# Stanford-ILIAD/Diverse-Conventions

Hardware: NVIDIA B200
Metric: agent-steps/sec (env+obs) (higher is better)
Workload: dtype u8

## Files before the change

diverse_conventions_b200/csrc/policy_kernels.cu:

```cuda
#include <cuda_bf16.h>
#include <cuda_runtime.h>
#include <stdint.h>
#include <stdlib.h>
#include <string.h>

#include <new>
#include <vector>

#include "api_common.h"
#include "oc_core.cuh"
#include "oc_device.cuh"
#include "mixed_schedule.h"
#include "ocb.h"
#include "policy_internal.h"

using namespace ocb;

namespace {

constexpr int kRows = 128;
constexpr int kHid = 64;
constexpr int kCo = 32;
constexpr int kSlots = 16;
constexpr int kK1 = 9 * kSlots;
// ... 480 lines not shown
                if (round > 0) mbar_wait_p<kProf>(bars + 8 * (PB_W_EMPTY + slot), (round - 1) & 1, pw[PW_W_EMPTY]);
                if (load) {
                    if (elect_one()) {
                        mbar_arrive_expect_tx(bars + 8 * (PB_W_FULL + slot), kChunk);
                        bulk_g2s(s_wring + slot * kChunk, (g ? blob_c : blob_a) + L.head_bytes + (size_t)j * kChunk, kChunk,
                                 bars + 8 * (PB_W_FULL + slot));
                    }
                    __syncwarp();
                }
                if (++slot == Reff) slot = 0, ++round;
            }
        }
    }
}

template <bool kProf, int kNet>
__device__ __forceinline__ void pair_conv_role(long long* pw, const PolicyParams& prm, int t0, int t1, const BlobLayout L, uint32_t tmem,
                                               uint32_t a_head, uint32_t bars, const int cp0 = 0, const int cpstep = 1,
                                               const uint32_t ring = kColRing, const int col_full = PB_COL_FULL,
                                               const int col_empty = PB_COL_EMPTY) {
    const int W = prm.W, H = prm.H, PH = H - 2, npos = prm.npos;
    constexpr int kN = kNet < 0 ? kHid : kCo;
    const uint32_t idesc = make_idesc(kRows, kN);
    const uint32_t a_wchi = a_head + (kNet == 1 ? kPConvBytes : 0), a_wclo = a_wchi + 2 * kPConvBytes;
    const int b_full = kNet < 0 ? PB_D1_FULL : PBS_D1_FULL + 2 * kNet, b_empty = kNet < 0 ? PB_D1_EMPTY : PBS_D1_EMPTY + 2 * kNet;
    uint32_t head_gen = 0, u = 0;
    uint32_t uses[2] = {0, 0};
    const bool tracer = kNet <= 0;
    uint32_t t_slot = 0, t_round = 0;
    auto advance = [&](uint32_t& slot, uint32_t& round, int n) {
        for (int i = 0; i < n; ++i)
            if (++slot == ring) slot = 0, ++round;
    };

    for (int t = t0; t < t1; ++t, ++u) {
        if (blob_changed(prm, t, t0)) {
            mbar_wait_p<kProf>(bars + 8 * PB_HEAD_FULL, head_gen & 1, pw[PW_HEAD_FULL]);
            ++head_gen;
        }
        if (kNet == 1) {
            const int s_last = (npos - 1) & 1;
            const uint32_t cum = (u + 1) * (uint32_t)((npos + 1 - s_last) / 2);
            mbar_wait_p<kProf>(bars + 8 * (PBS_D1_FULL + s_last), (cum - 1) & 1, pw[PW_D3_FULL]);
        }
        uint32_t w_slot = t_slot, w_round = t_round;
        uint32_t r_slot = t_slot;
        uint32_t c_slot = t_slot;
        int cols_seen = 0, released = 0, ox = 0, oy = cp0;
        while (oy >= PH) oy -= PH, ++ox, c_slot = (c_slot + 1 == ring) ? 0 : c_slot + 1;
        for (int cp = cp0; cp < npos; cp += cpstep) {
            const int st = cp & 1;
            for (; cols_seen < ox + 3; ++cols_seen) {
                mbar_wait_p<kProf>(bars + 8 * (col_full + w_slot), w_round & 1, pw[PW_COL_FULL]);
                if (++w_slot == ring) w_slot = 0, ++w_round;
// ... 7 lines not shown
            uint32_t n_slot = c_slot;
            while (noy >= PH) noy -= PH, ++nox, n_slot = (n_slot + 1 == ring) ? 0 : n_slot + 1;
            const int keep = cp + cpstep < npos ? nox : W;
            const uint32_t s1 = (c_slot + 1 >= ring) ? c_slot + 1 - ring : c_slot + 1;
            const uint32_t s2 = (c_slot + 2 >= ring) ? c_slot + 2 - ring : c_slot + 2;
            const uint32_t cellb = tmem + kColCells + (uint32_t)oy * kCellCols, colw = (uint32_t)H * kCellCols;
            const uint32_t cb0 = cellb + c_slot * colw, cb1 = cellb + s1 * colw, cb2 = cellb + s2 * colw;
            const long long ti0 = kProf ? clock64() : 0;
            if (cp == 3 && tracer) trace_ev<kProf>(prm, t - t0, 54);
            if (cp < 2 && tracer) trace_ev<kProf>(prm, t - t0, 11 + cp);
            if (elect_one()) {
#pragma unroll
                for (int j = 0; j < 9; ++j) {
                    const int dx = j / 3, dy = j - dx * 3;
                    const uint32_t ta = (dx == 0 ? cb0 : dx == 1 ? cb1 : cb2) + dy * kCellCols;
                    umma_bf16_ts(d1, ta, make_desc(a_wchi + j * 256, 128, 2304), idesc, j > 0);
                    umma_bf16_ts(d1, ta, make_desc(a_wclo + j * 256, 128, 2304), idesc, 1);
                }
                umma_commit(bars + 8 * (b_full + st));
                uint32_t rs = r_slot;
                for (int c = released; c < keep; ++c) {
                    umma_commit(bars + 8 * (col_empty + rs));
                    rs = (rs + 1 == ring) ? 0 : rs + 1;
                }
                if (cp + cpstep >= npos) umma_commit(bars + 8 * (PB_HEAD_EMPTY + (u & 1)));
            }
            __syncwarp();
            for (; released < keep; ++released) r_slot = (r_slot + 1 == ring) ? 0 : r_slot + 1;
            if (kProf) pw[PW_ISSUE_CONV] += clock64() - ti0;
            if (cp < 8 && tracer) trace_ev<kProf>(prm, t - t0, 16 + cp);
            ++uses[st];
            ox = nox, oy = noy, c_slot = n_slot;
// ... 142 lines not shown
            if (half == 1) {
                tc_fence_before();
                mbar_arrive(bars + 8 * (PB_D3_EMPTY + g));
            }
            head_accumulate(net, v, s_b2 + half * 32, s_wh, half * 32, head);
        }
        mbar_arrive(bars + 8 * (PB_HEAD_EMPTY + (u & 1)));
        if (kProf && (warp & 3) == 0) trace_ev<kProf>(prm, trace_vt, g == 0 ? 50 : 53);
        out(t, trow_id, net, head, drawn);
        if (kProf && warp == 0) trace_ev<kProf>(prm, trace_vt, 51);
    }
}
constexpr int kSColD3 = kPColD2 + kHid;
constexpr int kSHeadGroup = 1;

template <bool kProf>
__device__ __forceinline__ void single_fc_role(long long* pw, const PolicyParams& prm, int t0, int t1, const BlobLayout L, uint32_t tmem,
                                               uint32_t a_wring, uint32_t bars) {
    const int npos = prm.npos;
    const int R = prm.pair_ring, nch = L.chunks;
    const bool resident = R >= nch;
    const bool static_w = resident && prm.tile_policy == nullptr;
    const int Reff = resident ? nch : R;
    const uint32_t idesc = make_idesc(kRows, kHid);
    uint32_t u = 0, w_gen = 0, wround = 0;
    uint32_t cnt0 = 0, cnt1 = 0;
    int slot = 0;
    for (int t = t0; t < t1; ++t, ++u) {
        const bool chg = blob_changed(prm, t, t0);
        const bool w_loaded = !resident || chg;
        if (resident && w_loaded) ++w_gen;
        for (int j = 0; j < npos + 2; ++j) {
            const int sg = j < npos ? (j & 1) : (j - npos);
            const uint32_t k = sg ? cnt1 : cnt0;
            mbar_wait_p<kProf>(bars + 8 * (PB_A2_FULL + sg), k & 1, pw[PW_A2_FULL]);
            if (sg) ++cnt1; else ++cnt0;
            if (j == npos && u > 0) mbar_wait_p<kProf>(bars + 8 * PB_D3_EMPTY, (u - 1) & 1, pw[PW_D3_FULL]);
            if (w_loaded) mbar_wait_p<kProf>(bars + 8 * (PB_W_FULL + slot), resident ? ((w_gen - 1) & 1) : (wround & 1), pw[PW_W_FULL]);
            tc_fence_after();
            const uint32_t dst = tmem + (j < npos ? kPColD2 : kSColD3);
            const bool first = (j == 0 || j == npos);
            const uint32_t a_hi = tmem + kPColA2 + sg * kA2Cols, a_lo = a_hi + 16;
            const uint32_t b_hi = a_wring + slot * kChunk, b_lo = b_hi + 4096;
            const long long tf0 = kProf ? clock64() : 0;
            if (elect_one()) {
#pragma unroll
// ... 3 lines not shown
                    umma_bf16_ts(dst, a_hi + ks * 8, blo, idesc, 1);
                    umma_bf16_ts(dst, a_lo + ks * 8, bhi, idesc, 1);
                }
                umma_commit(bars + 8 * (PB_A2_EMPTY + sg));
                if (!static_w) umma_commit(bars + 8 * (PB_W_EMPTY + slot));
                if (j == npos - 1) umma_commit(bars + 8 * PB_D2_FULL);
                if (j == npos + 1) umma_commit(bars + 8 * PB_D3_FULL);
            }
            __syncwarp();
            if (kProf) pw[PW_ISSUE_FC] += clock64() - tf0;
            if (++slot >= Reff) slot = 0, ++wround;
        }
    }
}

template <bool kProf, class Out>
__device__ __forceinline__ void single_epilogue_role(long long* pw, const PolicyParams& prm, int t0, int t1, const BlobLayout L,
                                                     uint32_t tmem, const uint8_t* s_head, uint32_t bars, Out&& out) {
    const int warp = threadIdx.x >> 5, g = warp >> 2, trow_id = (warp & 3) * 32 + (threadIdx.x & 31);
    const int npos = prm.npos;
    const int net = prm.single == 2 ? 1 : 0;
    const uint32_t trow = tmem + ((uint32_t)((warp & 3) * 32) << 16);
    const uint8_t* rest = s_head + kPRestOff - L.bias1;
    const float* s_bias1 = reinterpret_cast<const float*>(rest + L.bias1);
    const float* s_b1 = reinterpret_cast<const float*>(rest + L.b1);
    const float* s_b2 = reinterpret_cast<const float*>(rest + L.b2);
    const float* s_wh = reinterpret_cast<const float*>(rest + L.wh);
    const float* s_bh = reinterpret_cast<const float*>(rest + L.bh);
    uint32_t u = 0, head_gen = 0, pubs = 0, d1_uses = 0;
    auto publish = [&](float (&v)[32], const float* bias) {
        const uint32_t a2 = trow + kPColA2 + g * kA2Cols;
        const float4* b4 = reinterpret_cast<const float4*>(bias);
        uint32_t hi[16], lo[16];
#pragma unroll
        for (int q = 0; q < 8; ++q) {
            const float4 b = b4[q];
            split2(fmaxf(v[4 * q] + b.x, 0.0f), fmaxf(v[4 * q + 1] + b.y, 0.0f), hi[2 * q], lo[2 * q]);
            split2(fmaxf(v[4 * q + 2] + b.z, 0.0f), fmaxf(v[4 * q + 3] + b.w, 0.0f), hi[2 * q + 1], lo[2 * q + 1]);
        }
        if (pubs >= 1) {
            mbar_wait_p<kProf>(bars + 8 * (PB_A2_EMPTY + g), (pubs - 1) & 1, pw[PW_A2_EMPTY]);
            tc_fence_after();
        }
        tmem_st16(a2, hi);
        tmem_st16(a2 + 16, lo);
        tmem_st_wait();
        tc_fence_before();
        mbar_arrive(bars + 8 * (PB_A2_FULL + g));
        ++pubs;
    };
    for (int t = t0; t < t1; ++t, ++u) {
        if (blob_changed(prm, t, t0)) {
            mbar_wait_p<kProf>(bars + 8 * PB_HEAD_FULL, head_gen & 1, pw[PW_HEAD_FULL]);
            ++head_gen;
        }
        for (int j = g; j < npos; j += 2, ++d1_uses) {
            mbar_wait_p<kProf>(bars + 8 * (PBS_D1_FULL + g), d1_uses & 1, pw[PW_D1_FULL]);
            tc_fence_after();
            float v[32];
            tmem_ld32(trow + kPColD1 + g * kCo, v);
            tc_fence_before();
            mbar_arrive(bars + 8 * (PBS_D1_EMPTY + g));
            publish(v, s_bias1 + j * kCo);
        }
        mbar_wait_p<kProf>(bars + 8 * PB_D2_FULL, u & 1, pw[PW_D2_FULL]);
        tc_fence_after();
        {
            float v[32];
            tmem_ld32(trow + kPColD2 + g * 32, v);
// ... 271 lines not shown
    }
    const int smem_max = kSmemBudget + 128;
    if (err == cudaSuccess) err = cudaFuncSetAttribute(policy_pair_kernel<false>, cudaFuncAttributeMaxDynamicSharedMemorySize, smem_max);
    if (err == cudaSuccess) err = cudaFuncSetAttribute(policy_pair_kernel<true>, cudaFuncAttributeMaxDynamicSharedMemorySize, smem_max);
    if (err == cudaSuccess) err = cudaFuncSetAttribute(rollout_fused_kernel<false, false, 1>, cudaFuncAttributeMaxDynamicSharedMemorySize, smem_max);
    if (err == cudaSuccess) err = cudaFuncSetAttribute(rollout_fused_kernel<true, false, 1>, cudaFuncAttributeMaxDynamicSharedMemorySize, smem_max);
    if (err == cudaSuccess) err = cudaFuncSetAttribute(rollout_fused_kernel<false, true, 1>, cudaFuncAttributeMaxDynamicSharedMemorySize, smem_max);
    if (err == cudaSuccess) err = cudaFuncSetAttribute(rollout_fused_kernel<true, true, 1>, cudaFuncAttributeMaxDynamicSharedMemorySize, smem_max);
    if (err == cudaSuccess) err = cudaFuncSetAttribute(rollout_fused_kernel<false, false, 2>, cudaFuncAttributeMaxDynamicSharedMemorySize, smem_max);
    if (err == cudaSuccess) err = cudaFuncSetAttribute(rollout_fused_kernel<true, false, 2>, cudaFuncAttributeMaxDynamicSharedMemorySize, smem_max);
    if (err == cudaSuccess) err = cudaFuncSetAttribute(rollout_fused_kernel<false, false, 1, true>, cudaFuncAttributeMaxDynamicSharedMemorySize, smem_max);
    if (err == cudaSuccess) err = cudaFuncSetAttribute(rollout_fused_kernel<false, true, 1, true>, cudaFuncAttributeMaxDynamicSharedMemorySize, smem_max);
    if (err == cudaSuccess) err = cudaFuncSetAttribute(rollout_fused_kernel<false, false, 2, true>, cudaFuncAttributeMaxDynamicSharedMemorySize, smem_max);
    if (err == cudaSuccess) err = cudaFuncSetAttribute(rollout_fused_kernel<false, false, 1, false, true>, cudaFuncAttributeMaxDynamicSharedMemorySize, smem_max);
    if (err == cudaSuccess) err = cudaFuncSetAttribute(rollout_fused_kernel<false, false, 2, false, true>, cudaFuncAttributeMaxDynamicSharedMemorySize, smem_max);
    if (err == cudaSuccess) err = cudaFuncSetAttribute(conv512_kernel, cudaFuncAttributeMaxDynamicSharedMemorySize, smem_max);
    if (err == cudaSuccess) err = cudaFuncSetAttribute(gemm512_kernel<false, false>, cudaFuncAttributeMaxDynamicSharedMemorySize, smem_max);
    if (err == cudaSuccess) err = cudaFuncSetAttribute(gemm512_kernel<true, true>, cudaFuncAttributeMaxDynamicSharedMemorySize, smem_max);
    if (err != cudaSuccess) {
        cudaGetLastError();
        ocb_policy_destroy(p);
        return fail(OCB_ERR_CUDA, "ocb_policy_create: %s", cudaGetErrorString(err));
    }
    *out = p;
    return OCB_OK;
}

static int set_weights512(ocb_policy* p, int policy, int net, const float* conv_w, const float* conv_b, const float* fc1_w,
                          const float* fc1_b, const float* fc2_w, const float* fc2_b, const float* head_w, const float* head_b) {
    const Blob5& L = p->L5;
// ... 355 lines not shown
    if (tile_policy == nullptr && (policy_index < 0 || policy_index >= p->n_policies)) return fail(OCB_ERR_INVALID_ARG, "policy index out of range");
    if (mixed && (mix->partner_policy < 0 || mix->partner_policy >= p->n_policies))
        return fail(OCB_ERR_INVALID_ARG, "policy index out of range");
    if (env_w != p->W || env_h != p->H) return fail(OCB_ERR_INVALID_ARG, "env and policy were built for different layouts");
    if (T < 1) return fail(OCB_ERR_INVALID_ARG, "T must be >= 1");
    if (mixed && (mix->L < 2 || T != 2 * mix->L || envp.N % (mix->L - 1) != 0))
        return fail(OCB_ERR_INVALID_ARG, "mixed play runs T = 2 L steps over a multiple of L - 1 worlds");
    if (mixed && (obs_slab == nullptr || actions == nullptr)) return fail(OCB_ERR_INVALID_ARG, "obs_buf and actions are required");
    if (!cross && !mixed && (obs_slab == nullptr || actions == nullptr || values == nullptr))
        return fail(OCB_ERR_INVALID_ARG, "obs_slab, actions and values are required");
    if (cross && (envp.N % kRows) != 0)
        return fail(OCB_ERR_INVALID_ARG, "cross-play needs a multiple of %d worlds (one weight set per 128-row tile of a seat), got %d", kRows, envp.N);
    if (population && (envp.N % kRows) != 0)
        return fail(OCB_ERR_INVALID_ARG, "population self-play needs a multiple of %d worlds (one weight set per slice), got %d", kRows, envp.N);
    if (cross && values != nullptr) return fail(OCB_ERR_INVALID_ARG, "the cross-play rollout runs no critic: values must be NULL");
    const int wtiles = (envp.N + kFWorlds - 1) / kFWorlds;
    int slots = 1;
    {
        const int fixed2 = fused_smem_layout(p->npos, 0, p->S, p->SC, 2).total;
        const bool fits2 = fixed2 <= kSmemBudget && (kSmemBudget - fixed2) / kChunk >= 4;
        const char* e = getenv("OCB_FUSED_SLOTS");
        const bool want2 = e != nullptr ? (e[0] == '2') : (wtiles > p->sm_count);
        if (want2 && fits2) slots = 2;
    }
    const int fixed = fused_smem_layout(p->npos, 0, p->S, p->SC, slots).total;
    int ring = (kSmemBudget - fixed) / kChunk;
    if (ring > kPMaxRing) ring = kPMaxRing;
    if (ring > 2 * p->L.chunks) ring = 2 * p->L.chunks;
    if (fixed > kSmemBudget || ring < 4)
        return fail(OCB_ERR_UNSUPPORTED, "layout too large for the fused rollout kernel (%d x %d)", p->W, p->H);
    DeviceGuard guard(p->device);
    FusedParams fp;
    memset(&fp, 0, sizeof(fp));
    fp.pol.blobs = tile_policy != nullptr ? p->d_blobs : p->d_blobs + (size_t)policy_index * 2 * (size_t)p->L.total;
    fp.pol.blob_stride = (size_t)p->L.total;
    fp.pol.W = p->W, fp.pol.H = p->H, fp.pol.S = p->S, fp.pol.SC = p->SC, fp.pol.npos = p->npos;
    fp.pol.M = kRows, fp.pol.tiles = 1;
    fp.pol.deterministic = deterministic, fp.pol.seed = seed, fp.pol.offset = 0;
    fp.pol.rng_rows_per_seat = p->rng_rows_per_seat, fp.pol.rng_add0 = p->rng_add0, fp.pol.rng_add1 = p->rng_add1;
    fp.pol.d_offset = reinterpret_cast<const unsigned long long*>(d_offset);
    fp.pol.net_mask = 3, fp.pol.pair_ring = ring, fp.pol.stage_stride = p->stage_stride;
    fp.pol.tile_policy = tile_policy, fp.pol.f_vt_round = slots * (T + 1), fp.pol.f_slots = slots;
    fp.pol.f_seat1_tiles = population ? 0 : envp.N / kRows;
    fp.env = envp;
    fp.T = T, fp.wtiles = wtiles, fp.slots = slots, fp.cross = cross ? 1 : 0;
    fp.obs_slab = obs_slab, fp.actions = actions, fp.logp = logp, fp.values = values, fp.reward = reward, fp.done = done;
    if (mixed) {
        fp.mix_L = mix->L, fp.mix_seed = mix->mix_seed, fp.mix_partner_seed = mix->partner_seed;
        fp.mix_partner_blobs = p->d_blobs + (size_t)mix->partner_policy * 2 * (size_t)p->L.total;
    }
    const int groups = (wtiles + slots - 1) / slots;
    const int ctas = groups < p->sm_count ? groups : p->sm_count;
    const size_t smem = (size_t)fused_smem_layout(p->npos, ring, p->S, p->SC, slots).total;
    fp.pol.trace = d_trace, fp.pol.trace_u0 = trace_u0, fp.pol.trace_n = trace_n;
    {
        const char* e = getenv("OCB_FUSED_VEC_LOADER");
        fp.vec_loader = e != nullptr ? (e[0] != '0') : (p->SC % 16 == 0);
    }
    {
        const int cols = 192 / (kCellCols * p->H);
        const char* e = getenv("OCB_FUSED_SPLIT");
        const bool want = e != nullptr ? (e[0] != '0') : true;
        fp.col_ring = (want && slots == 1 && !cross && !mixed && cols >= p->W) ? (p->W < kFMaxColRing ? p->W : kFMaxColRing) : 0;
        if (fp.col_ring < p->W) fp.col_ring = 0;
    }
    const cudaStream_t st = (cudaStream_t)stream;
    if (mixed) {
        fp.col_ring = kColRing;
        if (slots == 2)
            rollout_fused_kernel<false, false, 2, false, true><<<ctas, kFThreads, smem, st>>>(fp);
        else
            rollout_fused_kernel<false, false, 1, false, true><<<ctas, kFThreads, smem, st>>>(fp);
    } else if (population) {
        if (fp.col_ring > 0) {
            rollout_fused_kernel<false, true, 1, true><<<ctas, kFThreads, smem, st>>>(fp);
        } else {
            fp.col_ring = kColRing;
            if (slots == 2)
                rollout_fused_kernel<false, false, 2, true><<<ctas, kFThreads, smem, st>>>(fp);
            else
                rollout_fused_kernel<false, false, 1, true><<<ctas, kFThreads, smem, st>>>(fp);
        }
    } else if (fp.col_ring > 0) {
        if (d_trace != nullptr)
            rollout_fused_kernel<true, true, 1><<<ctas, kFThreads, smem, st>>>(fp);
        else
            rollout_fused_kernel<false, true, 1><<<ctas, kFThreads, smem, st>>>(fp);
// ... 22 lines not shown
```

diverse_conventions_b200/csrc/rollout_fused.cuh:

```cuda
#pragma once

struct FusedParams {
    PolicyParams pol;
    RolloutParams env;
    int T;
    int wtiles;
    int8_t* obs_slab;
    int32_t* actions;
    float* logp;
    float* values;
    int32_t* reward;
    int32_t* done;
    int vec_loader;
    int col_ring;
    int slots;
    int cross;
    int mix_L;
    unsigned long long mix_seed, mix_partner_seed;
    const uint8_t* mix_partner_blobs;
};

constexpr int kFEnvWarps = 2;
constexpr int kFWarpConvC = kPWarpProd + 1;
constexpr int kFWarpEnv = kFWarpConvC + 1;
constexpr int kFThreads = 32 * (kFWarpEnv + kFEnvWarps);
constexpr int kFWorlds = 32 * kFEnvWarps;
constexpr int kFMaxColRing = 6;
enum : int {
    FB_OBS_FULL = PB_COUNT,
    FB_OBS_EMPTY = PB_COUNT + 2,
    FB_ACT_FULL = PB_COUNT + 4,
    FB_COL_FULL = PB_COUNT + 6,
    FB_COL_EMPTY = FB_COL_FULL + kFMaxColRing,
    FB_COUNT = FB_COL_EMPTY + kFMaxColRing
};
static_assert((int)FB_COUNT <= (int)PB_TMEM_SLOT, "barrier block overflow");

struct FusedSmemLayout {
    int head, wring, bars, act, tables, tmpl, envw;
    int view_stride, env_warp_bytes, slot_bytes, total;
};
__host__ __device__ inline FusedSmemLayout fused_smem_layout(int npos, int ring, int S, int SC, int slots) {
// ... 26 lines not shown
    __device__ __forceinline__ void next() {
        if (two && s == 0) {
            s = 1;
            return;
        }
        s = 0;
        if (++u > T) u = 0, kt0 += stride, two = slots == 2 && kt0 + 1 < wtiles;
    }
};
__host__ __device__ inline int fused_virtual_tiles(int wtiles, int slots, int grid, int cta, int T) {
    int n = 0;
    for (int kt0 = cta * slots; kt0 < wtiles; kt0 += grid * slots) n += ((slots == 2 && kt0 + 1 < wtiles) ? 2 : 1) * (T + 1);
    return n;
}

template <bool kProf, bool kSplit>
__device__ __forceinline__ void fused_loader_role(const FusedParams& fp, uint32_t nvt, uint32_t tmem, const uint8_t* s_env,
                                                  const FusedSmemLayout& sl, uint32_t bars) {
    const int lwarp = (threadIdx.x >> 5) - kEpiWarps, lg = lwarp >> 2, lw = lwarp & 3, lane = threadIdx.x & 31;
    const int W = fp.pol.W, H = fp.pol.H, seg = 5 * H;
    const uint32_t* myrow0 = reinterpret_cast<const uint32_t*>(s_env + (lw & 1) * sl.env_warp_bytes + (lw >> 1) * sl.view_stride +
                                                               lane * fp.pol.SC);
    const uint32_t* myrow = myrow0;
    const uint32_t tcells = tmem + ((uint32_t)(lw * 32) << 16) + kColCells;
    const uint32_t ncols = nvt * (uint32_t)W;
    uint32_t lt = 0;
    int lx = lg;
    bool fresh = true;
    FusedCursor cur(fp);
    uint32_t seen[2] = {0, 0};
    for (uint32_t gc = lg; gc < ncols; gc += 2) {
        if (fresh) {
            myrow = myrow0 + cur.s * (sl.slot_bytes >> 2);
            mbar_wait(bars + 8 * (FB_OBS_FULL + cur.s), (cur.s ? seen[1] : seen[0]) & 1);
            if (kProf && lwarp == 0) trace_ev<kProf>(fp.pol, (int)lt, 8);
        }
        const bool first_col = fresh;
        fresh = false;
        const uint32_t ring = kSplit ? (uint32_t)fp.col_ring : (uint32_t)kColRing;
        const int slot = gc % ring;
        if (gc >= ring) {
            mbar_wait(bars + 8 * ((kSplit ? FB_COL_EMPTY : PB_COL_EMPTY) + slot), ((gc / ring) - 1) & 1);
            tc_fence_after();
        }
        if (fp.vec_loader) {
            const uint32_t* colp = myrow + lx * seg;
            const int r = (int)((reinterpret_cast<uintptr_t>(colp) >> 2) & 3);
            const uint4* src4 = reinterpret_cast<const uint4*>(colp - r);
            constexpr int kMaxVec = (5 * kMaxH + 3 + 3) / 4;
// ... 33 lines not shown
                for (int q = 0; q < 5; ++q) w[q] = mine[y * 5 + q];
                const uint4 c0 = make_uint4(bytes_bf16x2(w[0], pair_sel(0, 1)), bytes_bf16x2(w[0], pair_sel(2, 3)),
                                            bytes_bf16x2(w[1], pair_sel(0, 1)), bytes_bf16x2(w[1], pair_sel(2, 3)));
                const uint4 c1 = make_uint4(bytes_bf16x2(w[2], pair_sel(0, 1)), bytes_bf16x2(w[4], pair_sel(0, 1)),
                                            bytes_bf16x2(w[4], pair_sel(2, 3)), bytes_bf16x2(w[3], pair_sel(3, 4)));
                tmem_st8(tcells + (slot * H + y) * kCellCols, c0, c1);
            }
        }
        tmem_st_wait();
        tc_fence_before();
        mbar_arrive(bars + 8 * ((kSplit ? FB_COL_FULL : PB_COL_FULL) + slot));
        if (kProf && lwarp == 0 && first_col) trace_ev<kProf>(fp.pol, (int)lt, 9);
        if (kProf && lw == 0 && lx >= 1 && lx <= 4) trace_ev<kProf>(fp.pol, (int)lt, 3 + lx);
        lx += 2;
        if (lx >= W) {
            mbar_arrive(bars + 8 * (FB_OBS_EMPTY + cur.s));
            if (kProf && lwarp == 0) trace_ev<kProf>(fp.pol, (int)lt, 10);
            if (cur.s) ++seen[1]; else ++seen[0];
            cur.next();
            lx -= W, ++lt, fresh = true;
        }
    }
}

__device__ __forceinline__ void bulk_wait_read_1() { asm volatile("cp.async.bulk.wait_group.read 1;" ::: "memory"); }

template <int P>
struct FusedSlot {
    World<P> w;
    int cur_return, ep_add;
    long long ret_add;
    int n, nbytes;
    int j;
    bool valid, tma_ok, tma_pending;
    int8_t* obs_ptr;
    int32_t *rew_ptr, *done_ptr;
    uint32_t vts, acts;
};

template <bool kProf, int kSlots, bool kMix = false>
__device__ __forceinline__ void fused_env_role(const FusedParams& fp, uint8_t* s_env, const FusedSmemLayout& sl, const Tables& tb,
                                               const uint8_t* tmpl, const uint8_t* s_act, uint32_t bars) {
    constexpr int P = 2;
    const int ew = (threadIdx.x >> 5) - kFWarpEnv, lane = threadIdx.x & 31;
    const Consts c = load_consts(tb);
    const int SC = tb.SC, N = fp.env.N, T = fp.T;
    const int view_stride = sl.view_stride;
    const size_t PN = (size_t)P * N, obs_view_stride = (size_t)N * SC, obs_step_stride = PN * SC;
    const bool store_obs = fp.obs_slab != nullptr;

    FusedSlot<P> sa, sb;
    StepPre2 pre;
    sa.vts = sa.acts = sb.vts = sb.acts = 0;
    sa.tma_pending = sb.tma_pending = false;

    auto planes_of = [&](int slot) { return s_env + slot * sl.slot_bytes + ew * sl.env_warp_bytes; };
    auto objs_of = [&](int slot) { return reinterpret_cast<uint16_t*>(planes_of(slot) + (size_t)P * view_stride) + lane; };

    auto begin_tile = [&](FusedSlot<P>& q, int slot, int kt) {
        const int n0 = kt * kFWorlds + ew * 32;
        q.n = n0 + lane;
        q.valid = q.n < N;
        const int nl = q.valid ? q.n : N - 1;
        q.nbytes = max(0, min(32, N - n0)) * SC;
        q.obs_ptr = store_obs ? fp.obs_slab + (size_t)n0 * SC : nullptr;
        q.tma_ok = store_obs && fp.env.use_tma && q.nbytes > 0 && ((q.nbytes & 15) == 0) &&
                   ((reinterpret_cast<uintptr_t>(q.obs_ptr) & 15u) == 0) && ((obs_view_stride & 15u) == 0);
        q.rew_ptr = fp.reward ? fp.reward + q.n : nullptr;
        q.done_ptr = fp.done ? fp.done + q.n : nullptr;
        if constexpr (kMix) {
            q.j = q.n % (fp.mix_L - 1);
            q.tma_ok = store_obs && fp.env.use_tma && (SC & 15) == 0 && (reinterpret_cast<uintptr_t>(fp.obs_slab) & 15u) == 0;
        }
        load_world<P, 1, 8>(tb, c, fp.env, nl, 0, objs_of(slot), q.w);
        q.cur_return = fp.env.cur_return[nl];
// ... 14 lines not shown
                bulk_wait_read_all();
            } else if (lane == 0) {
                if (other_pending)
                    bulk_wait_read_1();
                else
                    bulk_wait_read_all();
            }
            q.tma_pending = false;
        }
        if (u > 0) {
            __syncwarp();
#pragma unroll
            for (int i = 0; i < P; ++i) oldslot[i] = q.w.slot[i];
            obs_phase1<P, 1>(tb, myplanes, view_stride, tmpl, false, 0, oldslot);
            mbar_wait(bars + 8 * (FB_ACT_FULL + slot), q.acts & 1);
            if (kProf && ew == 0) trace_ev<kProf>(fp.pol, (int)q.vts, 0);
            ++q.acts;
            int act[P];
            act[0] = s_act[slot * 128 + ew * 32 + lane], act[1] = s_act[slot * 128 + kFWorlds + ew * 32 + lane];
            int r;
            if constexpr (kSlots == 1)
                r = step_post(tb, c, q.w, myobjs, 32, act, pre, dirty, ticked);
            else
                r = step_world<P>(tb, c, q.w, myobjs, 32, act, dirty, ticked);
            const bool done = q.w.timestep >= c.horizon;
            q.cur_return += r;
            if (done) {
                q.ret_add += q.cur_return;
                q.ep_add += 1;
                q.cur_return = 0;
                reset_world<P>(tb, q.w);
                for (int idx = 0; idx < c.n_objcells; ++idx) myobjs[(int)tb.objcells[idx] * 32] = 0;
            }
            if constexpr (kMix) {
// ... 7 lines not shown
                    if (q.valid) q.rew_ptr[0] = r, q.rew_ptr[N] = r;
                    q.rew_ptr += PN;
                }
                if (q.done_ptr != nullptr) {
                    if (q.valid) *q.done_ptr = done ? 1 : 0;
                    q.done_ptr += N;
                }
            }
            full = done;
            if (kProf && ew == 0) trace_ev<kProf>(fp.pol, (int)q.vts, 1);
        }
        __syncwarp();
        if (kProf && ew == 0) trace_ev<kProf>(fp.pol, (int)q.vts, 2);
        if (full) obs_phase1<P, 1>(tb, myplanes, view_stride, tmpl, true, 0, oldslot);
        obs_phase2<P, 1>(tb, c, myplanes, view_stride, myobjs, 32, full, 0, q.w, dirty, ticked);
        mbar_arrive(bars + 8 * (FB_OBS_FULL + slot));
        if (kProf && ew == 0) trace_ev<kProf>(fp.pol, (int)q.vts, 3);
        ++q.vts;
        if (kMix && store_obs) {
            const bool rec = q.valid && u < T && mix_forced_main(fp.mix_L, u, q.j);
            int8_t* dst = rec ? fp.obs_slab + ((size_t)mix_record_slot(fp.mix_L, u, q.j) * PN + q.n) * SC : nullptr;
            if (q.tma_ok) {
                if (rec) {
                    fence_proxy_async_smem();
#pragma unroll
                    for (int v = 0; v < P; ++v)
                        bulk_store_s2g(dst + v * obs_view_stride, smem_addr(myplanes) + v * view_stride, (uint32_t)SC);
                    bulk_commit();
                }
                q.tma_pending = true;
            } else {
                __syncwarp();
                for (uint32_t todo = __ballot_sync(0xFFFFFFFFu, rec); todo != 0u; todo &= todo - 1u) {
// ... 43 lines not shown
        __syncwarp();
    };

    for (int kt0 = (int)blockIdx.x * kSlots; kt0 < fp.wtiles; kt0 += (int)gridDim.x * kSlots) {
        const bool two = kSlots == 2 && kt0 + 1 < fp.wtiles;
        begin_tile(sa, 0, kt0);
        if (kSlots == 2 && two) begin_tile(sb, 1, kt0 + 1);
        for (int u = 0; u <= T; ++u) {
            step_tile(sa, 0, u, kSlots == 2 && two && sb.tma_pending);
            if (kSlots == 2 && two) step_tile(sb, 1, u, sa.tma_pending);
        }
        end_tile(sa, 0);
        if (kSlots == 2 && two) end_tile(sb, 1);
    }
    if ((sa.tma_pending || (kSlots == 2 && sb.tma_pending)) && (kMix || lane == 0)) bulk_wait_read_all();
}

template <bool kMix = false>
struct FusedOut {
    const FusedParams& fp;
    uint8_t* s_act;
    uint32_t bars;
    unsigned long long base;
    FusedCursor cur;
    int g;
    bool partner_row;
    __device__ __forceinline__ FusedOut(const FusedParams& f, uint8_t* sa, uint32_t b) : fp(f), s_act(sa), bars(b), cur(f) {
        base = f.pol.offset;
        if (f.pol.d_offset != nullptr) base += *f.pol.d_offset;
        g = (int)(threadIdx.x >> 7);
// ... 37 lines not shown
            bool rec = valid;
            long long at = store;
            if constexpr (kMix) {
                const int j = valid ? n % (fp.mix_L - 1) : 0;
                rec = valid && g == 0 && mix_forced_main(fp.mix_L, u, j);
                at = ((long long)mix_record_slot(fp.mix_L, u, j) * 2 + seat) * N + n;
            }
            op.actions = rec ? fp.actions : nullptr, op.logp = rec ? fp.logp : nullptr, op.logits = nullptr;
            emit_actor_row(op, at, (uint32_t)row, head, base + (unsigned long long)u, true, &drawn, s_act + cur.s * 128 + trow_id,
                           bars + 8 * (FB_ACT_FULL + cur.s));
        }
        cur.next();
    }
};

template <bool kProf, bool kSplit, int kSlots, bool kPop = false, bool kMix = false>
__global__ void __launch_bounds__(kFThreads, 1) rollout_fused_kernel(const FusedParams fp) {
    extern __shared__ uint8_t smem_raw[];
    uint8_t* smem = smem_raw + ((128u - (smem_addr(smem_raw) & 127u)) & 127u);
    const int tid = threadIdx.x, warp = tid >> 5;
    const PolicyParams& prm = fp.pol;
    const BlobLayout L = blob_layout(prm.npos);
    const FusedSmemLayout sl = fused_smem_layout(prm.npos, prm.pair_ring, prm.S, prm.SC, fp.slots);
    uint8_t* s_head = smem + sl.head;
    uint8_t* s_wring = smem + sl.wring;
    uint64_t* s_bars = reinterpret_cast<uint64_t*>(smem + sl.bars);
    uint32_t* s_tmem = reinterpret_cast<uint32_t*>(s_bars + PB_TMEM_SLOT);
    uint8_t* s_act = smem + sl.act;
    Tables* s_tables = reinterpret_cast<Tables*>(smem + sl.tables);
    uint8_t* s_tmpl = smem + sl.tmpl;
    uint8_t* s_env = smem + sl.envw;
    const uint32_t bars = smem_addr(s_bars);

    if (warp == 0) {
        asm volatile("tcgen05.alloc.cta_group::1.sync.aligned.shared::cta.b32 [%0], %1;" ::"r"(smem_addr(s_tmem)),
                     "r"((uint32_t)kTmemCols)
                     : "memory");
        asm volatile("tcgen05.relinquish_alloc_permit.cta_group::1.sync.aligned;" ::: "memory");
    }
    if (tid == 32) {
        for (int i = 0; i < FB_COUNT; ++i) {
            uint32_t count = 1;
            if ((i >= PB_COL_FULL && i < PB_COL_FULL + 4) || (i >= PB_A2_FULL && i < PB_A2_FULL + 2) ||
                (i >= PB_D3_EMPTY && i < PB_D3_EMPTY + 2))
                count = 128;
            if (i >= PB_COL_EMPTY && i < PB_COL_EMPTY + 4) count = 2;
            if (i >= PB_HEAD_EMPTY && i < PB_HEAD_EMPTY + 2) count = 32 * kEpiWarps + (kSplit ? 3 : 2);
            if (i >= PB_D1_EMPTY && i < PB_D1_EMPTY + 2) count = 32 * kEpiWarps;
            if (i >= PBS_D1_EMPTY && i < PBS_D1_EMPTY + 4) count = 128;
            if (i >= FB_COL_FULL && i < FB_COL_FULL + kFMaxColRing) count = 128;
            if (i >= FB_COL_EMPTY && i < FB_COL_EMPTY + kFMaxColRing) count = 3;
            if (i >= FB_OBS_FULL && i < FB_OBS_FULL + 2) count = 32 * kFEnvWarps;
            if (i >= FB_OBS_EMPTY && i < FB_OBS_EMPTY + 2) count = 32 * kLoadWarps;
            if (i >= FB_ACT_FULL && i < FB_ACT_FULL + 2) count = 128;
            mbar_init(bars + 8 * i, count);
        }
        asm volatile("fence.mbarrier_init.release.cluster;" ::: "memory");
    }
    {
        const uint32_t* src = reinterpret_cast<const uint32_t*>(fp.env.tables);
        uint32_t* dst = reinterpret_cast<uint32_t*>(s_tables);
        for (int i = tid; i < (int)(sizeof(Tables) / 4); i += kFThreads) dst[i] = src[i];
        for (int i = tid; i < prm.SC; i += kFThreads) s_tmpl[i] = fp.env.tmpl[i];
    }
    tc_fence_before();
    __syncthreads();
    tc_fence_after();
    const uint32_t tmem = *s_tmem;
    const int nvt = fused_virtual_tiles(fp.wtiles, fp.slots, (int)gridDim.x, (int)blockIdx.x, fp.T);

    long long pw[kProf ? PW_COUNT : 1] = {};
    if (warp < kEpiWarps) {
        pair_epilogue_role<kProf, kSplit, kPop, kMix>(pw, prm, 0, nvt, L, tmem, s_head, bars, FusedOut<kMix>(fp, s_act, bars));
    } else if (warp < kWarpMma) {
        fused_loader_role<kProf, kSplit>(fp, (uint32_t)nvt, tmem, s_env, sl, bars);
    } else if (warp == kWarpMma || warp == kWarpConv2) {
        const int half = warp == kWarpMma ? 0 : 1;
        if (kSplit)
            pair_conv_role<kProf, 0>(pw, prm, 0, nvt, L, tmem, smem_addr(s_head), bars, half, 2, (uint32_t)fp.col_ring, FB_COL_FULL,
                                     FB_COL_EMPTY);
        else
            pair_conv_role<kProf, -1>(pw, prm, 0, nvt, L, tmem, smem_addr(s_head), bars, half, 2);
    } else if (warp == kPWarpProd) {
        pair_producer_role<kProf, kPop, kMix>(pw, prm, 0, nvt, L, smem_addr(s_head), smem_addr(s_wring), bars,
                                              kMix ? fp.mix_partner_blobs : nullptr);
    } else if (warp < kPWarpProd) {
        pair_fc_role<kProf, kSplit>(pw, prm, warp - kWarpFc, 0, nvt, L, tmem, smem_addr(s_wring), bars);
// ... 16 lines not shown
```

Measured before the change: 16.20 billion.

## Add seat-split fused cross-play rollout kernel with per-seat virtual tiles

Adds a new fused kernel variant for cross-play in which each tile of 128 worlds is processed as two virtual tiles, one per seat. Each virtual tile runs a single network, with seat-alternating weight offsets in the conv, FC and epilogue roles. A dedicated seat producer streams both partners' head and FC weights, and the env warps wait on both seats' actions before stepping. The aim is to replace the pair-network path, which computes both nets per tile, with a leaner single-net pipeline that gives better MMA utilisation. The cost is more complex barrier accounting, and each seat's observation pass is shared between two loader passes.

```diff
diff --git a/diverse_conventions_b200/csrc/policy_kernels.cu b/diverse_conventions_b200/csrc/policy_kernels.cu
--- a/diverse_conventions_b200/csrc/policy_kernels.cu
+++ b/diverse_conventions_b200/csrc/policy_kernels.cu
@@ -518,7 +518,7 @@
     }
 }
 
-template <bool kProf, int kNet>
+template <bool kProf, int kNet, bool kSeat = false>
 __device__ __forceinline__ void pair_conv_role(long long* pw, const PolicyParams& prm, int t0, int t1, const BlobLayout L, uint32_t tmem,
                                                uint32_t a_head, uint32_t bars, const int cp0 = 0, const int cpstep = 1,
                                                const uint32_t ring = kColRing, const int col_full = PB_COL_FULL,
@@ -542,6 +542,7 @@
             mbar_wait_p<kProf>(bars + 8 * PB_HEAD_FULL, head_gen & 1, pw[PW_HEAD_FULL]);
             ++head_gen;
         }
+        const uint32_t seat_w = kSeat ? (uint32_t)((t - t0) & 1) * kPConvBytes : 0u;
         if (kNet == 1) {
             const int s_last = (npos - 1) & 1;
             const uint32_t cum = (u + 1) * (uint32_t)((npos + 1 - s_last) / 2);
@@ -579,8 +580,8 @@
                 for (int j = 0; j < 9; ++j) {
                     const int dx = j / 3, dy = j - dx * 3;
                     const uint32_t ta = (dx == 0 ? cb0 : dx == 1 ? cb1 : cb2) + dy * kCellCols;
-                    umma_bf16_ts(d1, ta, make_desc(a_wchi + j * 256, 128, 2304), idesc, j > 0);
-                    umma_bf16_ts(d1, ta, make_desc(a_wclo + j * 256, 128, 2304), idesc, 1);
+                    umma_bf16_ts(d1, ta, make_desc(a_wchi + seat_w + j * 256, 128, 2304), idesc, j > 0);
+                    umma_bf16_ts(d1, ta, make_desc(a_wclo + seat_w + j * 256, 128, 2304), idesc, 1);
                 }
                 umma_commit(bars + 8 * (b_full + st));
                 uint32_t rs = r_slot;
@@ -753,11 +754,11 @@
 constexpr int kSColD3 = kPColD2 + kHid;
 constexpr int kSHeadGroup = 1;
 
-template <bool kProf>
+template <bool kProf, bool kSeat = false>
 __device__ __forceinline__ void single_fc_role(long long* pw, const PolicyParams& prm, int t0, int t1, const BlobLayout L, uint32_t tmem,
                                                uint32_t a_wring, uint32_t bars) {
     const int npos = prm.npos;
-    const int R = prm.pair_ring, nch = L.chunks;
+    const int R = prm.pair_ring, nch = (kSeat ? 2 : 1) * L.chunks;
     const bool resident = R >= nch;
     const bool static_w = resident && prm.tile_policy == nullptr;
     const int Reff = resident ? nch : R;
@@ -766,9 +767,10 @@
     uint32_t cnt0 = 0, cnt1 = 0;
     int slot = 0;
     for (int t = t0; t < t1; ++t, ++u) {
-        const bool chg = blob_changed(prm, t, t0);
+        const int ts = kSeat ? t - ((t - t0) & 1) : t;
+        const bool chg = blob_changed(prm, ts, t0);
         const bool w_loaded = !resident || chg;
-        if (resident && w_loaded) ++w_gen;
+        if (resident && w_loaded && ts == t) ++w_gen;
         for (int j = 0; j < npos + 2; ++j) {
             const int sg = j < npos ? (j & 1) : (j - npos);
             const uint32_t k = sg ? cnt1 : cnt0;
@@ -802,7 +804,7 @@
     }
 }
 
-template <bool kProf, class Out>
+template <bool kProf, bool kSeat = false, class Out>
 __device__ __forceinline__ void single_epilogue_role(long long* pw, const PolicyParams& prm, int t0, int t1, const BlobLayout L,
                                                      uint32_t tmem, const uint8_t* s_head, uint32_t bars, Out&& out) {
     const int warp = threadIdx.x >> 5, g = warp >> 2, trow_id = (warp & 3) * 32 + (threadIdx.x & 31);
@@ -816,6 +818,7 @@
     const float* s_wh = reinterpret_cast<const float*>(rest + L.wh);
     const float* s_bh = reinterpret_cast<const float*>(rest + L.bh);
     uint32_t u = 0, head_gen = 0, pubs = 0, d1_uses = 0;
+    const uint8_t* rest1 = rest + (L.head_bytes - L.bias1);
     auto publish = [&](float (&v)[32], const float* bias) {
         const uint32_t a2 = trow + kPColA2 + g * kA2Cols;
         const float4* b4 = reinterpret_cast<const float4*>(bias);
@@ -841,6 +844,12 @@
         if (blob_changed(prm, t, t0)) {
             mbar_wait_p<kProf>(bars + 8 * PB_HEAD_FULL, head_gen & 1, pw[PW_HEAD_FULL]);
             ++head_gen;
+        }
+        if constexpr (kSeat) {
+            const uint8_t* r = ((t - t0) & 1) ? rest1 : rest;
+            s_bias1 = reinterpret_cast<const float*>(r + L.bias1), s_b1 = reinterpret_cast<const float*>(r + L.b1);
+            s_b2 = reinterpret_cast<const float*>(r + L.b2), s_wh = reinterpret_cast<const float*>(r + L.wh);
+            s_bh = reinterpret_cast<const float*>(r + L.bh);
         }
         for (int j = g; j < npos; j += 2, ++d1_uses) {
             mbar_wait_p<kProf>(bars + 8 * (PBS_D1_FULL + g), d1_uses & 1, pw[PW_D1_FULL]);
@@ -1142,6 +1151,8 @@
     if (err == cudaSuccess) err = cudaFuncSetAttribute(rollout_fused_kernel<false, false, 2, true>, cudaFuncAttributeMaxDynamicSharedMemorySize, smem_max);
     if (err == cudaSuccess) err = cudaFuncSetAttribute(rollout_fused_kernel<false, false, 1, false, true>, cudaFuncAttributeMaxDynamicSharedMemorySize, smem_max);
     if (err == cudaSuccess) err = cudaFuncSetAttribute(rollout_fused_kernel<false, false, 2, false, true>, cudaFuncAttributeMaxDynamicSharedMemorySize, smem_max);
+    if (err == cudaSuccess) err = cudaFuncSetAttribute(rollout_fused_kernel<false, false, 1, false, false, true>, cudaFuncAttributeMaxDynamicSharedMemorySize, smem_max);
+    if (err == cudaSuccess) err = cudaFuncSetAttribute(rollout_fused_kernel<true, false, 1, false, false, true>, cudaFuncAttributeMaxDynamicSharedMemorySize, smem_max);
     if (err == cudaSuccess) err = cudaFuncSetAttribute(conv512_kernel, cudaFuncAttributeMaxDynamicSharedMemorySize, smem_max);
     if (err == cudaSuccess) err = cudaFuncSetAttribute(gemm512_kernel<false, false>, cudaFuncAttributeMaxDynamicSharedMemorySize, smem_max);
     if (err == cudaSuccess) err = cudaFuncSetAttribute(gemm512_kernel<true, true>, cudaFuncAttributeMaxDynamicSharedMemorySize, smem_max);
@@ -1527,16 +1538,17 @@
     if (population && (envp.N % kRows) != 0)
         return fail(OCB_ERR_INVALID_ARG, "population self-play needs a multiple of %d worlds (one weight set per slice), got %d", kRows, envp.N);
     if (cross && values != nullptr) return fail(OCB_ERR_INVALID_ARG, "the cross-play rollout runs no critic: values must be NULL");
-    const int wtiles = (envp.N + kFWorlds - 1) / kFWorlds;
+    const int fixed2 = fused_smem_layout(p->npos, 0, p->S, p->SC, 2).total;
+    const bool fits2 = fixed2 <= kSmemBudget && (kSmemBudget - fixed2) / kChunk >= 4;
+    const bool seat = cross && fits2;
+    const int wtiles = seat ? envp.N / kFSeatWorlds : (envp.N + kFWorlds - 1) / kFWorlds;
     int slots = 1;
-    {
-        const int fixed2 = fused_smem_layout(p->npos, 0, p->S, p->SC, 2).total;
-        const bool fits2 = fixed2 <= kSmemBudget && (kSmemBudget - fixed2) / kChunk >= 4;
+    if (!seat) {
         const char* e = getenv("OCB_FUSED_SLOTS");
         const bool want2 = e != nullptr ? (e[0] == '2') : (wtiles > p->sm_count);
         if (want2 && fits2) slots = 2;
     }
-    const int fixed = fused_smem_layout(p->npos, 0, p->S, p->SC, slots).total;
+    const int fixed = seat ? fixed2 : fused_smem_layout(p->npos, 0, p->S, p->SC, slots).total;
     int ring = (kSmemBudget - fixed) / kChunk;
     if (ring > kPMaxRing) ring = kPMaxRing;
     if (ring > 2 * p->L.chunks) ring = 2 * p->L.chunks;
@@ -1555,6 +1567,7 @@
     fp.pol.net_mask = 3, fp.pol.pair_ring = ring, fp.pol.stage_stride = p->stage_stride;
     fp.pol.tile_policy = tile_policy, fp.pol.f_vt_round = slots * (T + 1), fp.pol.f_slots = slots;
     fp.pol.f_seat1_tiles = population ? 0 : envp.N / kRows;
+    if (seat) fp.pol.single = 1, fp.pol.f_vt_round = 2 * T, fp.pol.f_slots = 2;
     fp.env = envp;
     fp.T = T, fp.wtiles = wtiles, fp.slots = slots, fp.cross = cross ? 1 : 0;
     fp.obs_slab = obs_slab, fp.actions = actions, fp.logp = logp, fp.values = values, fp.reward = reward, fp.done = done;
@@ -1564,7 +1577,7 @@
     }
     const int groups = (wtiles + slots - 1) / slots;
     const int ctas = groups < p->sm_count ? groups : p->sm_count;
-    const size_t smem = (size_t)fused_smem_layout(p->npos, ring, p->S, p->SC, slots).total;
+    const size_t smem = (size_t)fused_smem_layout(p->npos, ring, p->S, p->SC, seat ? 2 : slots).total;
     fp.pol.trace = d_trace, fp.pol.trace_u0 = trace_u0, fp.pol.trace_n = trace_n;
     {
         const char* e = getenv("OCB_FUSED_VEC_LOADER");
@@ -1584,6 +1597,12 @@
             rollout_fused_kernel<false, false, 2, false, true><<<ctas, kFThreads, smem, st>>>(fp);
         else
             rollout_fused_kernel<false, false, 1, false, true><<<ctas, kFThreads, smem, st>>>(fp);
+    } else if (seat) {
+        fp.col_ring = kColRing;
+        if (d_trace != nullptr)
+            rollout_fused_kernel<true, false, 1, false, false, true><<<ctas, kFThreads, smem, st>>>(fp);
+        else
+            rollout_fused_kernel<false, false, 1, false, false, true><<<ctas, kFThreads, smem, st>>>(fp);
     } else if (population) {
         if (fp.col_ring > 0) {
             rollout_fused_kernel<false, true, 1, true><<<ctas, kFThreads, smem, st>>>(fp);
diff --git a/diverse_conventions_b200/csrc/rollout_fused.cuh b/diverse_conventions_b200/csrc/rollout_fused.cuh
--- a/diverse_conventions_b200/csrc/rollout_fused.cuh
+++ b/diverse_conventions_b200/csrc/rollout_fused.cuh
@@ -26,6 +26,11 @@
 constexpr int kFThreads = 32 * (kFWarpEnv + kFEnvWarps);
 constexpr int kFWorlds = 32 * kFEnvWarps;
 constexpr int kFMaxColRing = 6;
+constexpr int kFSeatWorlds = 128;
+constexpr int kFSeatEnvWarps = 4;
+constexpr int kFWarpSeatEnv = kPWarpProd;
+constexpr int kFWarpSeatProd = kWarpFc + 1;
+static_assert(kFWarpSeatEnv + kFSeatEnvWarps == kFThreads / 32, "seat-tile env warps are the kernel's last four");
 enum : int {
     FB_OBS_FULL = PB_COUNT,
     FB_OBS_EMPTY = PB_COUNT + 2,
@@ -82,13 +87,14 @@
     return n;
 }
 
-template <bool kProf, bool kSplit>
+template <bool kProf, bool kSplit, bool kSeat = false>
 __device__ __forceinline__ void fused_loader_role(const FusedParams& fp, uint32_t nvt, uint32_t tmem, const uint8_t* s_env,
                                                   const FusedSmemLayout& sl, uint32_t bars) {
     const int lwarp = (threadIdx.x >> 5) - kEpiWarps, lg = lwarp >> 2, lw = lwarp & 3, lane = threadIdx.x & 31;
     const int W = fp.pol.W, H = fp.pol.H, seg = 5 * H;
-    const uint32_t* myrow0 = reinterpret_cast<const uint32_t*>(s_env + (lw & 1) * sl.env_warp_bytes + (lw >> 1) * sl.view_stride +
-                                                               lane * fp.pol.SC);
+    const uint32_t* myrow0 = reinterpret_cast<const uint32_t*>(
+        kSeat ? s_env + lw * sl.env_warp_bytes + lane * fp.pol.SC
+              : s_env + (lw & 1) * sl.env_warp_bytes + (lw >> 1) * sl.view_stride + lane * fp.pol.SC);
     const uint32_t* myrow = myrow0;
     const uint32_t tcells = tmem + ((uint32_t)(lw * 32) << 16) + kColCells;
     const uint32_t ncols = nvt * (uint32_t)W;
@@ -98,9 +104,10 @@
     FusedCursor cur(fp);
     uint32_t seen[2] = {0, 0};
     for (uint32_t gc = lg; gc < ncols; gc += 2) {
+        const bool seat1 = kSeat && (lt & 1u);
         if (fresh) {
-            myrow = myrow0 + cur.s * (sl.slot_bytes >> 2);
-            mbar_wait(bars + 8 * (FB_OBS_FULL + cur.s), (cur.s ? seen[1] : seen[0]) & 1);
+            myrow = myrow0 + (kSeat ? (seat1 ? (sl.view_stride >> 2) : 0) : cur.s * (sl.slot_bytes >> 2));
+            if (!seat1) mbar_wait(bars + 8 * (FB_OBS_FULL + cur.s), (cur.s ? seen[1] : seen[0]) & 1);
             if (kProf && lwarp == 0) trace_ev<kProf>(fp.pol, (int)lt, 8);
         }
         const bool first_col = fresh;
@@ -164,10 +171,12 @@
         if (kProf && lw == 0 && lx >= 1 && lx <= 4) trace_ev<kProf>(fp.pol, (int)lt, 3 + lx);
         lx += 2;
         if (lx >= W) {
-            mbar_arrive(bars + 8 * (FB_OBS_EMPTY + cur.s));
-            if (kProf && lwarp == 0) trace_ev<kProf>(fp.pol, (int)lt, 10);
-            if (cur.s) ++seen[1]; else ++seen[0];
-            cur.next();
+            if (!kSeat || seat1) {
+                mbar_arrive(bars + 8 * (FB_OBS_EMPTY + cur.s));
+                if (kProf && lwarp == 0) trace_ev<kProf>(fp.pol, (int)lt, 10);
+                if (cur.s) ++seen[1]; else ++seen[0];
+                cur.next();
+            }
             lx -= W, ++lt, fresh = true;
         }
     }
@@ -188,11 +197,12 @@
     uint32_t vts, acts;
 };
 
-template <bool kProf, int kSlots, bool kMix = false>
+template <bool kProf, int kSlots, bool kMix = false, bool kSeat = false>
 __device__ __forceinline__ void fused_env_role(const FusedParams& fp, uint8_t* s_env, const FusedSmemLayout& sl, const Tables& tb,
                                                const uint8_t* tmpl, const uint8_t* s_act, uint32_t bars) {
     constexpr int P = 2;
-    const int ew = (threadIdx.x >> 5) - kFWarpEnv, lane = threadIdx.x & 31;
+    constexpr int kTileWorlds = kSeat ? kFSeatWorlds : kFWorlds;
+    const int ew = (threadIdx.x >> 5) - (kSeat ? kFWarpSeatEnv : kFWarpEnv), lane = threadIdx.x & 31;
     const Consts c = load_consts(tb);
     const int SC = tb.SC, N = fp.env.N, T = fp.T;
     const int view_stride = sl.view_stride;
@@ -208,7 +218,7 @@
     auto objs_of = [&](int slot) { return reinterpret_cast<uint16_t*>(planes_of(slot) + (size_t)P * view_stride) + lane; };
 
     auto begin_tile = [&](FusedSlot<P>& q, int slot, int kt) {
-        const int n0 = kt * kFWorlds + ew * 32;
+        const int n0 = kt * kTileWorlds + ew * 32;
         q.n = n0 + lane;
         q.valid = q.n < N;
         const int nl = q.valid ? q.n : N - 1;
@@ -253,10 +263,14 @@
             for (int i = 0; i < P; ++i) oldslot[i] = q.w.slot[i];
             obs_phase1<P, 1>(tb, myplanes, view_stride, tmpl, false, 0, oldslot);
             mbar_wait(bars + 8 * (FB_ACT_FULL + slot), q.acts & 1);
+            if (kSeat) mbar_wait(bars + 8 * (FB_ACT_FULL + 1), q.acts & 1);
             if (kProf && ew == 0) trace_ev<kProf>(fp.pol, (int)q.vts, 0);
             ++q.acts;
             int act[P];
-            act[0] = s_act[slot * 128 + ew * 32 + lane], act[1] = s_act[slot * 128 + kFWorlds + ew * 32 + lane];
+            if (kSeat)
+                act[0] = s_act[ew * 32 + lane], act[1] = s_act[kFSeatWorlds + ew * 32 + lane];
+            else
+                act[0] = s_act[slot * 128 + ew * 32 + lane], act[1] = s_act[slot * 128 + kFWorlds + ew * 32 + lane];
             int r;
             if constexpr (kSlots == 1)
                 r = step_post(tb, c, q.w, myobjs, 32, act, pre, dirty, ticked);
@@ -294,9 +308,11 @@
         if (kProf && ew == 0) trace_ev<kProf>(fp.pol, (int)q.vts, 2);
         if (full) obs_phase1<P, 1>(tb, myplanes, view_stride, tmpl, true, 0, oldslot);
         obs_phase2<P, 1>(tb, c, myplanes, view_stride, myobjs, 32, full, 0, q.w, dirty, ticked);
-        mbar_arrive(bars + 8 * (FB_OBS_FULL + slot));
-        if (kProf && ew == 0) trace_ev<kProf>(fp.pol, (int)q.vts, 3);
-        ++q.vts;
+        if (!kSeat || u < T) {
+            mbar_arrive(bars + 8 * (FB_OBS_FULL + slot));
+            if (kProf && ew == 0) trace_ev<kProf>(fp.pol, (int)q.vts, 3);
+            ++q.vts;
+        }
         if (kMix && store_obs) {
             const bool rec = q.valid && u < T && mix_forced_main(fp.mix_L, u, q.j);
             int8_t* dst = rec ? fp.obs_slab + ((size_t)mix_record_slot(fp.mix_L, u, q.j) * PN + q.n) * SC : nullptr;
@@ -370,6 +386,54 @@
         if (kSlots == 2 && two) end_tile(sb, 1);
     }
     if ((sa.tma_pending || (kSlots == 2 && sb.tma_pending)) && (kMix || lane == 0)) bulk_wait_read_all();
+}
+
+template <bool kProf>
+__device__ __forceinline__ void seat_producer_role(long long* pw, const PolicyParams& prm, int nvt, const BlobLayout L, uint32_t s_head,
+                                                   uint32_t s_wring, uint32_t bars) {
+    const int R = prm.pair_ring, nch = 2 * L.chunks;
+    const bool resident = R >= nch;
+    const int Reff = resident ? nch : R;
+    const uint32_t rest = (uint32_t)(L.head_bytes - L.bias1);
+    uint32_t round = 0;
+    int slot = 0;
+    bool chg = false;
+    const uint8_t* blob[2] = {prm.blobs, prm.blobs};
+    for (int t = 0; t < nvt; ++t) {
+        const int seat = t & 1;
+        if (seat == 0) {
+            chg = blob_changed(prm, t, 0);
+            const uint32_t tp = fused_pair(prm, t);
+            blob[0] = prm.blobs + (size_t)(tp & 0xFFFFu) * 2 * prm.blob_stride;
+            blob[1] = prm.blobs + (size_t)(tp >> 16) * 2 * prm.blob_stride;
+            if (chg) {
+                if (t > 0) mbar_wait_p<kProf>(bars + 8 * (PB_HEAD_EMPTY + ((t - 1) & 1)), ((t - 1) >> 1) & 1, pw[PW_HEAD_EMPTY]);
+                if (elect_one()) {
+                    const uint32_t hb = bars + 8 * PB_HEAD_FULL;
+                    mbar_arrive_expect_tx(hb, 2u * (2u * kPConvBytes + rest));
+#pragma unroll
+                    for (int g = 0; g < 2; ++g) {
+                        bulk_g2s(s_head + g * kPConvBytes, blob[g] + L.wc_hi, kPConvBytes, hb);
+                        bulk_g2s(s_head + (2 + g) * kPConvBytes, blob[g] + L.wc_lo, kPConvBytes, hb);
+                        bulk_g2s(s_head + kPRestOff + g * rest, blob[g] + L.bias1, rest, hb);
+                    }
+                }
+                __syncwarp();
+            }
+        }
+        const bool load = !resident || chg;
+        for (int j = 0; j < L.chunks; ++j) {
+            if (round > 0) mbar_wait_p<kProf>(bars + 8 * (PB_W_EMPTY + slot), (round - 1) & 1, pw[PW_W_EMPTY]);
+            if (load) {
+                if (elect_one()) {
+                    mbar_arrive_expect_tx(bars + 8 * (PB_W_FULL + slot), kChunk);
+                    bulk_g2s(s_wring + slot * kChunk, blob[seat] + L.head_bytes + (size_t)j * kChunk, kChunk, bars + 8 * (PB_W_FULL + slot));
+                }
+                __syncwarp();
+            }
+            if (++slot == Reff) slot = 0, ++round;
+        }
+    }
 }
 
 template <bool kMix = false>
@@ -437,14 +501,42 @@
     }
 };
 
-template <bool kProf, bool kSplit, int kSlots, bool kPop = false, bool kMix = false>
+struct FusedSeatOut {
+    const FusedParams& fp;
+    uint8_t* s_act;
+    uint32_t bars;
+    unsigned long long base;
+    int kt, u, seat;
+    __device__ __forceinline__ FusedSeatOut(const FusedParams& f, uint8_t* sa, uint32_t b) : fp(f), s_act(sa), bars(b) {
+        base = f.pol.offset;
+        if (f.pol.d_offset != nullptr) base += *f.pol.d_offset;
+        kt = (int)blockIdx.x, u = 0, seat = 0;
+    }
+    __device__ __forceinline__ uint32_t draw(int, int trow_id) const {
+        if (fp.pol.deterministic) return 0u;
+        return policy_draw(fp.pol, (uint32_t)(seat * fp.env.N + kt * kFSeatWorlds + trow_id), base + (unsigned long long)u);
+    }
+    __device__ __forceinline__ void operator()(int, int trow_id, int, const float (&head)[6], uint32_t drawn) {
+        const long long row = (long long)seat * fp.env.N + (kt * kFSeatWorlds + trow_id);
+        PolicyParams op = fp.pol;
+        op.actions = fp.actions, op.logp = fp.logp, op.logits = nullptr;
+        emit_actor_row(op, (long long)u * 2 * fp.env.N + row, (uint32_t)row, head, base + (unsigned long long)u, true, &drawn,
+                       s_act + seat * kFSeatWorlds + trow_id, bars + 8 * (FB_ACT_FULL + seat));
+        if (++seat == 2) {
+            seat = 0;
+            if (++u >= fp.T) u = 0, kt += (int)gridDim.x;
+        }
+    }
+};
+
+template <bool kProf, bool kSplit, int kSlots, bool kPop = false, bool kMix = false, bool kSeat = false>
 __global__ void __launch_bounds__(kFThreads, 1) rollout_fused_kernel(const FusedParams fp) {
     extern __shared__ uint8_t smem_raw[];
     uint8_t* smem = smem_raw + ((128u - (smem_addr(smem_raw) & 127u)) & 127u);
     const int tid = threadIdx.x, warp = tid >> 5;
     const PolicyParams& prm = fp.pol;
     const BlobLayout L = blob_layout(prm.npos);
-    const FusedSmemLayout sl = fused_smem_layout(prm.npos, prm.pair_ring, prm.S, prm.SC, fp.slots);
+    const FusedSmemLayout sl = fused_smem_layout(prm.npos, prm.pair_ring, prm.S, prm.SC, kSeat ? 2 : fp.slots);
     uint8_t* s_head = smem + sl.head;
     uint8_t* s_wring = smem + sl.wring;
     uint64_t* s_bars = reinterpret_cast<uint64_t*>(smem + sl.bars);
@@ -473,7 +565,7 @@
             if (i >= PBS_D1_EMPTY && i < PBS_D1_EMPTY + 4) count = 128;
             if (i >= FB_COL_FULL && i < FB_COL_FULL + kFMaxColRing) count = 128;
             if (i >= FB_COL_EMPTY && i < FB_COL_EMPTY + kFMaxColRing) count = 3;
-            if (i >= FB_OBS_FULL && i < FB_OBS_FULL + 2) count = 32 * kFEnvWarps;
+            if (i >= FB_OBS_FULL && i < FB_OBS_FULL + 2) count = 32 * (kSeat ? kFSeatEnvWarps : kFEnvWarps);
             if (i >= FB_OBS_EMPTY && i < FB_OBS_EMPTY + 2) count = 32 * kLoadWarps;
             if (i >= FB_ACT_FULL && i < FB_ACT_FULL + 2) count = 128;
             mbar_init(bars + 8 * i, count);
@@ -490,10 +582,24 @@
     __syncthreads();
     tc_fence_after();
     const uint32_t tmem = *s_tmem;
-    const int nvt = fused_virtual_tiles(fp.wtiles, fp.slots, (int)gridDim.x, (int)blockIdx.x, fp.T);
+    const int nvt = kSeat ? 2 * fused_virtual_tiles(fp.wtiles, 1, (int)gridDim.x, (int)blockIdx.x, fp.T - 1)
+                          : fused_virtual_tiles(fp.wtiles, fp.slots, (int)gridDim.x, (int)blockIdx.x, fp.T);
 
     long long pw[kProf ? PW_COUNT : 1] = {};
-    if (warp < kEpiWarps) {
+    if (kSeat) {
+        if (warp < kEpiWarps)
+            single_epilogue_role<kProf, true>(pw, prm, 0, nvt, L, tmem, s_head, bars, FusedSeatOut(fp, s_act, bars));
+        else if (warp < kWarpMma)
+            fused_loader_role<kProf, false, true>(fp, (uint32_t)nvt, tmem, s_env, sl, bars);
+        else if (warp == kWarpMma || warp == kWarpConv2)
+            pair_conv_role<kProf, 0, true>(pw, prm, 0, nvt, L, tmem, smem_addr(s_head), bars, warp == kWarpMma ? 0 : 1, 2);
+        else if (warp == kWarpFc)
+            single_fc_role<kProf, true>(pw, prm, 0, nvt, L, tmem, smem_addr(s_wring), bars);
+        else if (warp == kFWarpSeatProd)
+            seat_producer_role<kProf>(pw, prm, nvt, L, smem_addr(s_head), smem_addr(s_wring), bars);
+        else
+            fused_env_role<kProf, 1, false, true>(fp, s_env, sl, *s_tables, s_tmpl, s_act, bars);
+    } else if (warp < kEpiWarps) {
         pair_epilogue_role<kProf, kSplit, kPop, kMix>(pw, prm, 0, nvt, L, tmem, s_head, bars, FusedOut<kMix>(fp, s_act, bars));
     } else if (warp < kWarpMma) {
         fused_loader_role<kProf, kSplit>(fp, (uint32_t)nvt, tmem, s_env, sl, bars);
```

After: 16.21 billion (median of 6 runs). Within noise of the previous version (+0.0%).
